# agwi-lab/renderformer

Hardware: AMD Instinct MI355X
Metric: rendered frames/sec at 512×512, renderformer-v1.1-swin-large, 1/2/4/8 MI355X (higher is better)
Workload: dtype fp16+bf16

## Files before the change

### renderformer_amd/csrc/gemm.hip

```cpp
#include <algorithm>
#include <type_traits>
#include <cmath>
#include <math.h>
#include <stdio.h>
#include <stdlib.h>
#include <string.h>

#include "common.h"
#include "env.h"

namespace {

constexpr int BK = 32;
constexpr int P_F16 = 2;

enum Epi { E_BF16 = RF_EPI_BF16, E_F32 = RF_EPI_F32, E_ADD = RF_EPI_ADD_F32, E_SWIGLU = RF_EPI_SWIGLU, E_CONV = 16,
           E_ROPE = 17 };

template <int BM_, int BN_, int WGM_, int WGN_, int STAGES_, int KH_ = 1>
struct Tile {
    static constexpr int BM = BM_, BN = BN_, WGM = WGM_, WGN = WGN_, STAGES = STAGES_, KH = KH_;
    static constexpr int NWAVE = WGM * WGN, THREADS = NWAVE * 64;
    static constexpr int MW = BM / WGM, NWD = BN / WGN, TI = MW / 16, TJ = NWD / 16;
    static constexpr int APIECES = BM / 16;
// ... 1790 lines not shown
            wait_vm<0>();
            __syncthreads();
            if (kf == 0) pn_issue<C, EPI>(p, area, m0, n0);
            engine_mainloop<C, NTERM, GATHER, EPI == E_ADD>(p, smem, m0, n0, kf, kl, acc);
            if (kf != 0) {
                const __amdgpu_buffer_rsrc_t rs = __builtin_amdgcn_make_buffer_rsrc(
                    p.sk_part + (int64_t)L * (BM * BN), 0, BM * BN * 4, 0x00020000);
#pragma unroll
                for (int i = 0; i < TI; ++i)
#pragma unroll
                    for (int j = 0; j < TJ; ++j) {
                        const int off = (((wave * TI + i) * TJ + j) * 64 + lane) * 16;
                        __builtin_amdgcn_raw_buffer_store_b128(__builtin_bit_cast(u32x4, acc[i][j]), rs, off, 0, 16);
                    }
                asm volatile("s_waitcnt vmcnt(0)" ::: "memory");
                __syncthreads();
                if (threadIdx.x == 0) __hip_atomic_store(p.sk_flag + L, p.sk_epoch, __ATOMIC_RELAXED, __HIP_MEMORY_SCOPE_AGENT);
            } else {
                if (kl < iters) {
                    const int64_t tile_end = (int64_t)(tile + 1) * iters;
                    for (int c = L + 1; c < gend; ++c) {
                        int64_t cb, ce;
                        lay.equal_range(c, grp, ntiles64, iters, cb, ce);
                        if (cb >= tile_end) break;
                        if (ce == cb) continue;
                        if (threadIdx.x == 0) {
                            int spins = 0;
                            while (__hip_atomic_load(p.sk_flag + c, __ATOMIC_RELAXED, __HIP_MEMORY_SCOPE_AGENT) != p.sk_epoch &&
                                   ++spins < p.spin)
                                __builtin_amdgcn_s_sleep(1);
                            if (spins >= p.spin) report_device_error(p.err, RF_DEVERR_SK_GEMM);
                            __builtin_amdgcn_fence(__ATOMIC_ACQUIRE, "agent");
                            asm volatile("s_waitcnt vmcnt(0)" ::: "memory");
                        }
                        __syncthreads();
                        const float4* src =
                            reinterpret_cast<const float4*>(p.sk_part + (int64_t)c * (BM * BN)) + wave * TI * TJ * 64 + lane;
#pragma unroll
                        for (int i = 0; i < TI; ++i)
#pragma unroll
                            for (int j = 0; j < TJ; ++j) {
                                const float4 v = src[(i * TJ + j) * 64];
                                acc[i][j][0] += v.x;
                                acc[i][j][1] += v.y;
                                acc[i][j][2] += v.z;
                                acc[i][j][3] += v.w;
                            }
                    }
                }
                engine_epilogue<C, EPI>(p, m0, n0, acc, area);
            }
            it += kl - kf;
        }
    }
}

constexpr int GROUP_MAX = 4;
struct GroupArgs {
    EngineArgs p[GROUP_MAX];
    int first[GROUP_MAX + 1];
    int n;
};

template <class C, int EPI, int NTERM, bool GATHER>
__global__ __launch_bounds__(C::THREADS, 2) void engine_group_kernel(GroupArgs g) {
    constexpr int BM = C::BM, BN = C::BN, TI = C::TI, TJ = C::TJ;
    __shared__ __attribute__((aligned(16))) char smem[C::STAGES * stage_bytes<C, NTERM>()];
    const int nwg = gridDim.x, hw = blockIdx.x;
    const int xcd = hw & 7, qd = nwg >> 3, rd = nwg & 7;
    const int wg = (xcd < rd ? xcd * (qd + 1) : rd * (qd + 1) + (xcd - rd) * qd) + (hw >> 3);
    int q = 0;
#pragma unroll
    for (int i = 1; i < GROUP_MAX; ++i) q += (i < g.n && wg >= g.first[i]) ? 1 : 0;
    const EngineArgs& p = g.p[q];
    const int local = wg - g.first[q];
    const int tiles_m = (p.m + BM - 1) / BM;
    int tm, tn;
    tile_coords(local, tiles_m, p.n / BN, p.group_m, tm, tn);
    f32x4 acc[TI][TJ];
    engine_mainloop<C, NTERM, GATHER, EPI == E_ADD>(p, smem, tm * BM, tn * BN, 0, p.k / (BK * C::KH), acc);
    engine_epilogue<C, EPI>(p, tm * BM, tn * BN, acc);
}

template <class C>
struct Halo {
    static constexpr int ROWS = (3 * (C::BM + 2) + 15) / 16 * 16;
    static constexpr int BYTES = ROWS * 64;
    static constexpr int PIECES = ROWS / 16;
    static constexpr int PPW = (PIECES + C::NWAVE - 1) / C::NWAVE;
    static constexpr int BST = 3;
    static constexpr int LDS = 2 * BYTES + BST * C::B_BYTES;
};

template <class C>
RF_DEV void halo_mainloop(const EngineArgs& p, char* smem, int m0, int n0, f32x4 (&acc)[C::TI][C::TJ]) {
    using H = Halo<C>;
    constexpr int TI = C::TI, TJ = C::TJ, PB = C::PB, S = H::BST;
    const int lane = threadIdx.x & 63;
    const int wave = threadIdx.x >> 6;
    const int wm = wave / C::WGN, wn = wave % C::WGN;
    const int lg = p.halo_lg, tw = 1 << lg, hw2 = tw + 2;
    const int hr_n = ((C::BM >> lg) + 2) * hw2;
    const int per_img = p.ho * p.wo;
    const int img = m0 / per_img, rem = m0 - img * per_img;
    const int y0 = rem / p.wo, x0 = rem - y0 * p.wo;

    int hpix[H::PPW];
#pragma unroll
    for (int t = 0; t < H::PPW; ++t) {
        const int hr = (wave + C::NWAVE * t) * 16 + (lane >> 2);
        int pix = -1;
        if (hr < hr_n) {
            const int hy = hr / hw2, hx = hr - hy * hw2;
            const int iy = y0 + hy - 1, ix = x0 + hx - 1;
            if (iy >= 0 && iy < p.hi && ix >= 0 && ix < p.wi) pix = (img * p.hi + iy) * p.wi + ix;
        }
        hpix[t] = pix;
    }
    int brow[PB], blc[PB];
#pragma unroll
    for (int pc = 0; pc < PB; ++pc) {
        brow[pc] = (wave * PB + pc) * 16 + (lane >> 2);
        blc[pc] = (lane & 3) ^ ((brow[pc] >> 1) & 3);
    }
    auto issue_halo = [&](int chunk, int buf) {
#pragma unroll
        for (int t = 0; t < H::PPW; ++t) {
            const int piece = wave + C::NWAVE * t;
            if (piece < H::PIECES) {
                const int hch = (lane & 3) ^ (((piece * 16 + (lane >> 2)) >> 1) & 3);
                const bf16_t* src = hpix[t] >= 0 ? p.a + (int64_t)hpix[t] * p.cin_pad + chunk * BK + hch * 8 : p.zero;
                __builtin_amdgcn_global_load_lds(GLB_PTR(void, src), LDS_PTR(void, smem + buf * H::BYTES + piece * 1024),
                                                 16, 0, 0);
            }
        }
    };
    auto issue_w = [&](int kt, int stage) {
        const int chunk = kt / 9, tap = kt - 9 * chunk;
        const int k0 = tap * p.cin_pad + chunk * BK;
        char* st = smem + 2 * H::BYTES + stage * C::B_BYTES;
#pragma unroll
        for (int pc = 0; pc < PB; ++pc) {
            const int piece = wave * PB + pc;
            const int64_t woff = (int64_t)(n0 + brow[pc]) * p.ldw + k0 + blc[pc] * 8;
            __builtin_amdgcn_global_load_lds(GLB_PTR(void, p.w + woff), LDS_PTR(void, st + piece * 1024), 16, 0, 0);
        }
    };

#pragma unroll
    for (int i = 0; i < TI; ++i)
#pragma unroll
        for (int j = 0; j < TJ; ++j) acc[i][j] = f32x4{0.f, 0.f, 0.f, 0.f};

    const int nch = p.cin_pad / BK, nk = 9 * nch;
    const int frag_row = lane & 15, frag_ch = lane >> 4;
    auto base_hr = [&](int i) {
        const int r = wm * C::MW + i * 16 + frag_row;
        return r + ((r >> lg) << 1);
    };
    struct Frags {
        bf16x8 a[TI], w[TJ];
    };
    auto load_frags = [&](int kt, Frags& f) {
        const int chunk = kt / 9, tap = kt - 9 * chunk;
        const int ky = tap / 3, kx = tap - 3 * ky;
        const char* hb = smem + (chunk & 1) * H::BYTES;
// ... 762 lines not shown
    RF_LAUNCH((engine_kernel<C, EPI, NTERM, GATHER, true>), dim3(grid), dim3(C::THREADS), 0,
                       (hipStream_t)stream, a);
    return rf::check_launch(what);
}

int sk_setup(EngineArgs& p, void* workspace, void* stream) {
    p.sk_part = (float*)workspace;
    p.sk_flag = (int*)(p.sk_part + SK_PART_FLOATS);
    p.sk_epoch = rf::next_epoch(p.sk_flag, SK_MAX_GRID * sizeof(int), (hipStream_t)stream);
    if (p.sk_epoch == 0) return RF_ERR_LAUNCH;
    p.err = rf::device_error_word();
    p.spin = rf::spin_limit();
    p.stamps = RF_ENV_ONCE("RF_GEMM_STAMPS", 0) != 0 ? (uint64_t*)(p.sk_part + SK_PART_FLOATS - 65536) : nullptr;
    return RF_OK;
}

template <class F>
int with_epi(int epilogue, F&& f) {
    switch (epilogue) {
        case RF_EPI_BF16: return f(std::integral_constant<int, E_BF16>{});
        case RF_EPI_F32: return f(std::integral_constant<int, E_F32>{});
        case RF_EPI_ADD_F32: return f(std::integral_constant<int, E_ADD>{});
        default: return f(std::integral_constant<int, E_SWIGLU>{});
    }
}

inline void dense_args(EngineArgs& p, const void* a, int64_t lda, const void* w, int64_t ldw, int m, int n, int k,
                       void* c, int64_t ldc) {
    p.a = (const bf16_t*)a;
    p.lda = lda;
    p.w = (const bf16_t*)w;
    p.ldw = ldw;
    p.m = m;
    p.n = n;
    p.k = k;
    p.c = c;
    p.ldc = ldc;
}


int sk_grid(int m, int n, int k) {
    const bool env = rf::env_set("RF_GEMM_SK");
    int grid = 2 * 256;
    if (!env) return 0;
    if (env) {
        grid = rf::env_int("RF_GEMM_SK", 0);
        if (grid <= 0) return 0;
        grid = grid > SK_MAX_GRID ? SK_MAX_GRID : grid;
    }
    const int64_t tiles = (int64_t)((m + 127) / 128) * (n / 128);
    const int64_t rounds = (tiles + 511) / 512;
    const double eff = (double)tiles / (rounds * 512);
    if (!env && (eff >= 0.9 || tiles * (k / BK) < 8LL * grid)) return 0;
    return grid;
}

enum TileCode : int {
    TC_R128 = 128,
    TC_P256 = 256,
    TC_P288 = 288,
    TC_R64 = 642,
    TC_P64 = 643,
    TC_R64w4 = 644,
    TC_P3_64 = 645,
    TC_R64s6 = 646,
    TC_R96 = 962,
    TC_P96 = 963,
    TC_P3_96 = 964,
    TC_R96s5 = 965,
    TC_R96s6 = 966,
    TC_P128 = 1282,
    TC_P3_128 = 1283,
    TC_R128s4 = 1284,
    TC_R128s5 = 1285,
    TC_R128s6 = 1286,
    TC_R128w8s6 = 1288,
    TC_R256x128 = 2561,
    TC_R64k2 = 6423,
    TC_R64w4k2 = 6443,
    TC_R96k2 = 9623,
    TC_R128k2s3 = 12823,
    TC_R128k2s4 = 12824,
    TC_R128w8k2 = 12884,
};

int pick_cfg(int m, int n, int k, int epilogue = RF_EPI_BF16) {
    if (rf::env_set("RF_GEMM_TILE")) return rf::env_int("RF_GEMM_TILE", 0);
    const bool phased = n % 256 == 0 && k % 64 == 0 && rf::env_int("RF_GEMM_PHASED", 1) != 0;
    const double kk = k / 1024.0;
    const bool add = epilogue == RF_EPI_ADD_F32;
    auto cost = [&](int bm, int bn, int slots, double fixed, double per_k, double add_cost) {
        const int64_t tiles = (int64_t)((m + bm - 1) / bm) * (n / bn);
        const int64_t rounds = (tiles + 256 * slots - 1) / (256 * slots);
        return rounds * (fixed + per_k * kk + (add ? add_cost : 0.0));
    };
    int best = TC_R128;
    const int64_t t128 = (int64_t)((m + 127) / 128) * (n / 128);
    double best_c = t128 <= 256 ? cost(128, 128, 1, 5.5, 13.1, 5.0) : cost(128, 128, 2, 11.0, 14.0, 5.0);
    auto consider = [&](int cfg, double c) {
        if (c < best_c) {
            best_c = c;
            best = cfg;
        }
    };
    if (k % 64 == 0) consider(TC_R128w8k2, cost(128, 128, 1, 6.8, 10.9, 5.0));
    if (n % 256 == 0) consider(TC_R96, cost(96, 256, 1, 2.2, 16.5, 13.0));
    if (phased) {
        consider(TC_P256, cost(256, 256, 1, 11.0, 20.4, 5.0));
        consider(TC_P288, cost(288, 256, 1, 22.5, 22.1, 5.0));
        consider(TC_P128, cost(128, 256, 1, 2.3, 18.4, 5.0));
        consider(TC_P3_96, cost(96, 256, 1, 6.0, 14.4, 5.0));
        consider(TC_P3_64, cost(64, 256, 1, 6.5, 11.8, 5.0));
    }
    return best;
}

__device__ __attribute__((aligned(16))) bf16_t g_zero_row[64];

namespace mx {
constexpr int BM = 256, BN = 256, KS = 128;
constexpr int A_DATA = BM * KS, B_DATA = BN * KS;
constexpr int STAGE = A_DATA + B_DATA + (BM + BN) * 4;
constexpr int TI = 8, TJ = 4;
typedef __attribute__((ext_vector_type(8))) int i32x8;
RF_DEV int off(int row, int ch) { return row * KS + ((ch ^ (row & 7)) << 4); }
}

template <bool INITC>
RF_DEV void mx8_mainloop(const EngineArgs& p, char* smem, int m0, int n0, int kbeg, int kend,
                         f32x4 (&acc)[mx::TI][mx::TJ]) {
    using namespace mx;
    const int lane = threadIdx.x & 63;
    const int wave = threadIdx.x >> 6;
    const int wm = wave >> 2, wn = wave & 3;
    const int nk = kend - kbeg;
    const uint8_t* A = reinterpret_cast<const uint8_t*>(p.a);
    const uint8_t* W = reinterpret_cast<const uint8_t*>(p.w);
    auto issue = [&](int kt, int buf) {
        char* st = smem + buf * STAGE;
        const int64_t k0 = (int64_t)(kbeg + kt) * KS;
#pragma unroll
        for (int i = 0; i < 8; ++i) {
            const int piece = wave * 8 + i;
            const bool is_a = piece < BM / 8;
            const int row = (is_a ? piece : piece - BM / 8) * 8 + (lane >> 3);
            const int ch = (lane & 7) ^ (row & 7);
            const uint8_t* src;
            if (is_a) {
                const int m = m0 + row;
                src = A + (int64_t)(m < p.m ? m : p.m - 1) * p.lda + k0 + ch * 16;
            } else {
                src = W + (int64_t)(n0 + row) * p.ldw + k0 + ch * 16;
            }
            __builtin_amdgcn_global_load_lds(GLB_PTR(void, src), LDS_PTR(void, st + (is_a ? 0 : A_DATA) + piece % (BM / 8) * 1024),
                                             16, 0, 0);
        }
        {
            const bool is_a = wave < BM / 64;
            const int row = (is_a ? wave : wave - BM / 64) * 64 + lane;
            const uint8_t* src;
            if (is_a) {
                const int m = m0 + row;
                src = p.sa + (int64_t)(m < p.m ? m : p.m - 1) * p.ld_sa + (kbeg + kt) * 4;
            } else {
                src = p.sw + (int64_t)(n0 + row) * p.ld_sw + (kbeg + kt) * 4;
            }
            __builtin_amdgcn_global_load_lds(GLB_PTR(void, src),
                                             LDS_PTR(void, st + A_DATA + B_DATA + (is_a ? 0 : BM * 4) + (row & ~63) * 4),
                                             4, 0, 0);
        }
    };
    if (INITC && kbeg == 0) {
        load_c_acc<TI, TJ>(p, m0 + wm * 128, n0 + wn * 64, acc);
    } else {
#pragma unroll
        for (int i = 0; i < TI; ++i)
#pragma unroll
            for (int j = 0; j < TJ; ++j) acc[i][j] = f32x4{0.f, 0.f, 0.f, 0.f};
    }
    const int frow = lane & 15, g = lane >> 4;
    issue(0, 0);
    if (nk > 1) {
        issue(1, 1);
        wait_vm<9>();
    } else {
        wait_vm<0>();
    }
    __builtin_amdgcn_s_barrier();
// ... 217 lines not shown
    int e = -127;
    if (amax > 0.f) {
        int ex;
        const float f = frexpf(amax, &ex);
        e = ex - 9 + (f > 0.875f ? 1 : 0);
        e = e < -127 ? -127 : (e > 127 ? 127 : e);
    }
    const float inv = ldexpf(1.0f, -e);
    uint32_t out[8];
#pragma unroll
    for (int i = 0; i < 8; ++i) {
        int pk = __builtin_amdgcn_cvt_pk_fp8_f32(v[4 * i] * inv, v[4 * i + 1] * inv, 0, false);
        pk = __builtin_amdgcn_cvt_pk_fp8_f32(v[4 * i + 2] * inv, v[4 * i + 3] * inv, pk, true);
        out[i] = (uint32_t)pk;
    }
    uint4* dst = reinterpret_cast<uint4*>(q + (int64_t)row * ldq + b * 32);
    dst[0] = make_uint4(out[0], out[1], out[2], out[3]);
    dst[1] = make_uint4(out[4], out[5], out[6], out[7]);
    sc[(int64_t)row * lds + b] = (uint8_t)(e + 127);
}

}

bool persist_on() {
    return RF_ENV_ONCE("RF_GEMM_PERSIST", 1) != 0;
}

bool persist_ragged() {
    return RF_ENV_ONCE("RF_GEMM_PERSIST_RAGGED", 0) != 0;
}

template <int EPI, int NTERM, bool GATHER, int BM = 256>
int launch_phased(EngineArgs a, void* stream, const char* what) {
    const int tiles_m = (a.m + BM - 1) / BM, tiles_n = a.n / 256;
    const int nwg = tiles_n * tiles_m;
    a.group_m = pick_group_m(tiles_m, tiles_n, BM, 256, (nwg + 7) / 8, GATHER ? 0 : (int64_t)a.m * a.k * 2);
    if constexpr (BM == 256 && (NTERM == 1 || NTERM == P_F16) && !GATHER) {
        if (nwg > 256 && persist_on() && (nwg % 256 == 0 || persist_ragged())) {
            a.persist = 1;
            RF_LAUNCH((phased_sk_kernel<EPI, NTERM>), dim3(256), dim3(512), 0, (hipStream_t)stream, a);
            return rf::check_launch(what);
        }
    }
    RF_LAUNCH((phased_kernel<BM, EPI, NTERM, GATHER>), dim3(nwg), dim3(512), 0, (hipStream_t)stream, a);
    return rf::check_launch(what);
}

#ifdef RF_STUDY
int l2pf_dist() {
    return std::max(0, std::min(8, rf::env_int("RF_GEMM_L2PF", 0)));
}
#endif

template <int EPI, int BM, int NT = 1>
int launch_phased3(EngineArgs a, void* stream, const char* what) {
#ifdef RF_STUDY
    a.l2pf = l2pf_dist();
#endif
    const int tiles_m = (a.m + BM - 1) / BM, tiles_n = a.n / 256;
    const int nwg = tiles_n * tiles_m;
    a.group_m = pick_group_m(tiles_m, tiles_n, BM, 256, (nwg + 7) / 8, (int64_t)a.m * a.k * 2);
    RF_LAUNCH((phased3_kernel<BM, EPI, NT>), dim3(nwg), dim3(512), 0, (hipStream_t)stream, a);
    return rf::check_launch(what);
}

template <int EPI, int NT = 1>
int launch_phased_sk(EngineArgs a, int grid, void* stream, const char* what) {
    const int tiles_m = (a.m + 255) / 256, tiles_n = a.n / 256;
    a.group_m = pick_group_m(tiles_m, tiles_n, 256, 256, ((int64_t)tiles_m * tiles_n + 7) / 8);
    RF_LAUNCH((phased_sk_kernel<EPI, NT>), dim3(grid), dim3(512), 0, (hipStream_t)stream, a);
    return rf::check_launch(what);
}

bool use_phased(int n, int k) {
    return rf::env_int("RF_GEMM_PHASED", 1) != 0 && n % 256 == 0 && k % 64 == 0;
}

template <class C>
struct Ring {};
template <int BM>
struct Phased {};
template <int BM>
struct Phased3 {};

enum Pre { PRE_NONE = 0, PRE_N256 = 1, PRE_K64 = 2, PRE_PHASED = 4 };

bool pre_ok(int pre, const EngineArgs& p) {
    return (!(pre & PRE_N256) || p.n % 256 == 0) && (!(pre & PRE_K64) || p.k % 64 == 0) &&
           (!(pre & PRE_PHASED) || use_phased(p.n, p.k));
}

template <int CODE, class LOOP, int PRE, bool F16>
struct Row {};
template <class... R>
struct Rows {};

using TileTable = Rows<
    Row<TC_P256,        Phased<256>,                      PRE_PHASED,          true>,
    Row<TC_P128,        Phased<128>,                      PRE_PHASED,          true>,
    Row<TC_P288,        Phased<288>,                      PRE_PHASED,          true>,
    Row<TC_P256,        Ring<T256>,                       PRE_N256,            false>,
    Row<TC_R128s4,      Ring<Tile<128, 128, 2, 2, 4>>,    PRE_NONE,            false>,
    Row<TC_R128s5,      Ring<Tile<128, 128, 2, 2, 5>>,    PRE_NONE,            false>,
    Row<TC_R256x128,    Ring<T256x128>,                   PRE_NONE,            false>,
    Row<TC_R96,         Ring<T96x256>,                    PRE_N256,            true>,
    Row<TC_R64,         Ring<T64x256>,                    PRE_N256,            false>,
    Row<TC_P3_128,      Phased3<128>,                     PRE_PHASED,          true>,
    Row<TC_P3_96,       Phased3<96>,                      PRE_PHASED,          true>,
    Row<TC_P3_64,       Phased3<64>,                      PRE_PHASED,          true>,
    Row<TC_P96,         Phased<96>,                       PRE_PHASED,          false>,
    Row<TC_P64,         Phased<64>,                       PRE_PHASED,          false>,
    Row<TC_R64w4,       Ring<T64x256w4>,                  PRE_N256,            false>,
    Row<TC_R96s5,       Ring<T96x256s5>,                  PRE_N256,            false>,
    Row<TC_R96s6,       Ring<T96x256s6>,                  PRE_N256,            false>,
    Row<TC_R64s6,       Ring<T64x256s6>,                  PRE_N256,            false>,
    Row<TC_R128s6,      Ring<T128s6>,                     PRE_NONE,            false>,
    Row<TC_R128w8s6,    Ring<T128w8s6>,                   PRE_NONE,            false>,
    Row<TC_R128k2s3,    Ring<T128k2s3>,                   PRE_K64,             false>,
    Row<TC_R128k2s4,    Ring<T128k2s4>,                   PRE_K64,             false>,
    Row<TC_R128w8k2,    Ring<T128w8k2s4>,                 PRE_K64,             true>,
    Row<TC_R96k2,       Ring<T96x256k2>,                  PRE_K64 | PRE_N256,  false>,
    Row<TC_R64k2,       Ring<T64x256k2>,                  PRE_K64 | PRE_N256,  false>,
    Row<TC_R64w4k2,     Ring<T64x256w4k2>,                PRE_K64 | PRE_N256,  false>,
    Row<TC_R128,        Ring<T128>,                       PRE_NONE,            true>>;

template <int NT, class C>
int run_loop(Ring<C>, const EngineArgs& p, int epilogue, void* stream) {
    return with_epi(epilogue, [&](auto e) { return launch<C, decltype(e)::value, NT>(p, stream, "rf_gemm"); });
}
template <int NT, int BM>
int run_loop(Phased<BM>, const EngineArgs& p, int epilogue, void* stream) {
    return with_epi(epilogue, [&](auto e) {
        return launch_phased<decltype(e)::value, NT, false, BM>(p, stream, NT == P_F16 ? "rf_gemm_f16" : "rf_gemm_bf16");
    });
}
template <int NT, int BM>
int run_loop(Phased3<BM>, const EngineArgs& p, int epilogue, void* stream) {
    return with_epi(epilogue, [&](auto e) { return launch_phased3<decltype(e)::value, BM, NT>(p, stream, "rf_gemm"); });
}

template <int NT, int CODE, class LOOP, int PRE, bool F16>
bool try_row(Row<CODE, LOOP, PRE, F16>, int cfg, const EngineArgs& p, int epilogue, void* stream, int& rc) {
    if constexpr (NT == P_F16 && !F16) {
        return false;
    } else {
        if (cfg != CODE || !pre_ok(PRE, p)) return false;
        rc = run_loop<NT>(LOOP{}, p, epilogue, stream);
        return true;
    }
}

template <int NT, class... R>
int run_dp(Rows<R...>, int cfg, const EngineArgs& p, int epilogue, void* stream) {
    int rc = RF_OK;
    if ((try_row<NT>(R{}, cfg, p, epilogue, stream, rc) || ...)) return rc;
    return run_loop<NT>(Ring<T128>{}, p, epilogue, stream);
}

bool sk256(int m, int n, int k) { return rf::env_int("RF_GEMM_SK256", 0) != 0; }

bool skph(int m, int n, int k) {
    if (!use_phased(n, k)) return false;
    if (rf::env_set("RF_GEMM_SKPH")) return rf::env_int("RF_GEMM_SKPH", 0) != 0;
    const int64_t tiles = (int64_t)((m + 255) / 256) * (n / 256);
    return n % 256 == 0 && tiles >= 512 && tiles % 256 == 0;
}

extern "C" int64_t rf_gemm_workspace_bytes(void) { return SK_WS_BYTES; }

#ifdef RF_STUDY
static int quad_tile() {
    const char* env = rf::env_str("RF_GEMM_QUAD_TILE");
    if (!env) return 256256;
    int bm = 0, bn = 0;
    if (sscanf(env, "%dx%d", &bm, &bn) != 2) return 256256;
    return bm * 1000 + bn;
}

static int quad_mode(int m, int n, int k, int64_t lda, int64_t ldw, int epilogue) {
    const int mode = rf::env_int("RF_GEMM_QUAD", 0);
    if (mode <= 0 || k % 128 || m <= 0) return 0;
    const int t = quad_tile(), bn = t % 1000;
    if (bn != 256 && bn != 192 && bn != 128) return 0;
    if (epilogue == RF_EPI_SWIGLU && n % bn) return 0;
    if ((int64_t)m * lda * 2 >= 0x7fffffff || (int64_t)n * ldw * 2 >= 0x7fffffff) return 0;
    return mode;
}

template <int WM, int WN, int EPI, int NT, int STG>
static int launch_quad_s(EngineArgs a, int mode, void* workspace, int64_t ws_bytes, void* stream, const char* what);

template <int WM, int WN, int EPI, int NT>
static int launch_quad(EngineArgs a, int mode, void* workspace, int64_t ws_bytes, void* stream, const char* what) {
    if (rf::env_int("RF_GEMM_QUAD_STG", 0) == 1) return launch_quad_s<WM, WN, EPI, NT, 1>(a, mode, workspace, ws_bytes, stream, what);
    return launch_quad_s<WM, WN, EPI, NT, 0>(a, mode, workspace, ws_bytes, stream, what);
}

template <int WM, int WN, int EPI, int NT, int STG>
static int launch_quad_s(EngineArgs a, int mode, void* workspace, int64_t ws_bytes, void* stream, const char* what) {
    using G = qd::Cfg<WM, WN>;
    const int tiles_m = (a.m + G::BM - 1) / G::BM, tiles_n = (a.n + G::BN - 1) / G::BN;
    const int64_t tiles = (int64_t)tiles_m * tiles_n;
    const int grid = (int)std::min<int64_t>(tiles, 256);
    a.group_m = pick_group_m(tiles_m, tiles_n, G::BM, G::BN, (grid + 7) / 8);
    if (mode == 2 && workspace && ws_bytes >= SK_WS_BYTES) {
        if (const int rc = sk_setup(a, workspace, stream)) return rc;
        RF_LAUNCH((quad_kernel<WM, WN, EPI, NT, STG>), dim3(256), dim3(256), 0, (hipStream_t)stream, a);
    } else {
        a.sk_flag = nullptr;
        RF_LAUNCH((quad_kernel<WM, WN, EPI, NT, STG>), dim3(grid), dim3(256), 0, (hipStream_t)stream, a);
    }
    return rf::check_launch(what);
}

template <int WM, int WN, int NT>
static int run_quad_t(const EngineArgs& p, int epilogue, int mode, void* workspace, int64_t ws_bytes, void* stream,
                      const char* what) {
    return with_epi(epilogue, [&](auto e) {
        return launch_quad<WM, WN, decltype(e)::value, NT>(p, mode, workspace, ws_bytes, stream, what);
    });
}
// ... 98 lines not shown
    nio.xg = (bf16_t*)xg;
    nio.ldxg = ldxg;
    nio.norm_g = norm_w;
    nio.ss_out = ss;
    nio.xg_f16 = f16;
    return gemm_bf16(a, lda, w, ldw, x, ldx, nullptr, m, n, k, RF_EPI_ADD_F32, workspace, ws_bytes, stream, nullptr,
                     f16, &nio);
}

extern "C" int rf_gemm_rownorm(const void* a, int64_t lda, const void* w, int64_t ldw, void* c, int64_t ldc, int m,
                               int n, int k, int epilogue, const float* ss, int norm_dim, float eps, float* seg_ss,
                               int seg_w, int n_seg, int operand_dtype, void* workspace, int64_t ws_bytes,
                               void* stream) {
    RF_REQUIRE(ss && ((uintptr_t)ss & 15) == 0, "rf_gemm_rownorm: ss must be 16-B aligned");
    RF_REQUIRE(norm_dim > 0, "rf_gemm_rownorm: norm_dim must be positive");
    RF_REQUIRE(epilogue == RF_EPI_BF16 || epilogue == RF_EPI_F16 || epilogue == RF_EPI_SWIGLU ||
                   epilogue == RF_EPI_SWIGLU_F16,
               "rf_gemm_rownorm: epilogue must be RF_EPI_BF16 / F16 / SWIGLU / SWIGLU_F16 (got %d)", epilogue);
    RF_REQUIRE(operand_dtype == RF_DT_F16 || operand_dtype == RF_DT_BF16, "rf_gemm_rownorm: operand_dtype");
    RF_REQUIRE(!seg_ss || ((epilogue == RF_EPI_BF16 || epilogue == RF_EPI_F16) && ((uintptr_t)seg_ss & 15) == 0 &&
                           seg_w > 0 && seg_w % 256 == 0 && seg_w <= PN_SLOTS * 128 && n_seg >= 1 &&
                           (int64_t)seg_w * n_seg <= n),
               "rf_gemm_rownorm: seg_ss needs a 16-bit (non-SwiGLU) epilogue, 16-B alignment, seg_w %% 256 == 0 and "
               "<= %d, n_seg >= 1 segments inside N", PN_SLOTS * 128);
    EngineArgs nio{};
    nio.rs_part = ss;
    nio.rs_n = (float)norm_dim;
    nio.rs_eps = eps;
    nio.seg_ss = seg_ss;
    nio.seg_w = seg_w;
    nio.seg_n = seg_ss ? n_seg : 0;
    return gemm_bf16(a, lda, w, ldw, c, ldc, nullptr, m, n, k, epilogue, workspace, ws_bytes, stream, nullptr,
                     operand_dtype == RF_DT_F16, &nio);
}

template <class C, int NT>
static int launch_rope(EngineArgs p, void* stream) {
    return launch<C, E_ROPE, NT>(p, stream, "rf_gemm_qk_rope");
}

extern "C" int rf_gemm_qk_rope(const void* a, int64_t lda, const void* w, int64_t ldw, void* c, int64_t ldc, int m,
                               int n, int k, const float* ss, int norm_dim, float eps, float* seg_ss, int seg_w,
                               int n_seg, const float* norm_w, const float* pos, int64_t ld_pos, int pos_div,
                               const float* freqs, int n_freqs, float q_scale, int operand_dtype, void* workspace,
                               int64_t ws_bytes, void* stream) {
    (void)workspace;
    (void)ws_bytes;
    RF_REQUIRE(a && w && c, "rf_gemm_qk_rope: null pointer");
    RF_REQUIRE(m > 0 && n > 0 && k > 0, "rf_gemm_qk_rope: empty problem m=%d n=%d k=%d", m, n, k);
    RF_REQUIRE(operand_dtype == RF_DT_F16 || operand_dtype == RF_DT_BF16, "rf_gemm_qk_rope: operand_dtype");
    RF_REQUIRE(k % 64 == 0 && n % 128 == 0, "rf_gemm_qk_rope: needs K %% 64 == 0 and N %% 128 == 0");
    RF_REQUIRE(lda % 8 == 0 && ldw % 8 == 0 && lda >= k && ldw >= k && ((uintptr_t)a & 15) == 0 &&
                   ((uintptr_t)w & 15) == 0, "rf_gemm_qk_rope: operands must be 16-B aligned with lda/ldw >= K");
    RF_REQUIRE(ldc >= n && ldc % 4 == 0 && ((uintptr_t)c & 7) == 0, "rf_gemm_qk_rope: ldc too small/unaligned");
    RF_REQUIRE(seg_w > 0 && seg_w % 256 == 0 && seg_w % 128 == 0 && n_seg >= 1 && (int64_t)seg_w * n_seg <= n,
               "rf_gemm_qk_rope: the q/k segments must be whole 256-column tiles inside N");
    RF_REQUIRE(!seg_ss || (((uintptr_t)seg_ss & 15) == 0 && seg_w <= PN_SLOTS * 128),
               "rf_gemm_qk_rope: seg_ss must be 16-B aligned and seg_w <= %d", PN_SLOTS * 128);
    RF_REQUIRE(!ss || (((uintptr_t)ss & 15) == 0 && norm_dim > 0), "rf_gemm_qk_rope: ss must be 16-B aligned");
    RF_REQUIRE(!norm_w || ((uintptr_t)norm_w & 15) == 0, "rf_gemm_qk_rope: norm_w must be 16-B aligned");
    RF_REQUIRE(!pos || (freqs && n_freqs > 0 && 9 * n_freqs <= 64 && ld_pos >= 9 && pos_div >= 1),
               "rf_gemm_qk_rope: pos needs freqs with 9 * n_freqs <= 64, ld_pos >= 9 and pos_div >= 1");
    EngineArgs p{};
    dense_args(p, a, lda, w, ldw, m, n, k, c, ldc);
    p.rs_part = ss;
    p.rs_n = (float)norm_dim;
    p.rs_eps = eps;
    p.seg_ss = norm_w ? seg_ss : nullptr;
    p.seg_w = seg_w;
    p.seg_n = n_seg;
    p.rope_pos = pos;
    p.rope_ld = ld_pos;
    p.rope_div = pos ? pos_div : 1;
    p.rope_freqs = freqs;
    p.rope_nf = pos ? n_freqs : 1;
    p.rope_g = norm_w;
    p.rope_qscale = q_scale;
    const bool f16 = operand_dtype == RF_DT_F16;
    const int cfg = pick_cfg(m, n, k, RF_EPI_BF16);
    if (cfg == TC_P288 && use_phased(n, k)) {
        return f16 ? launch_phased<E_ROPE, P_F16, false, 288>(p, stream, "rf_gemm_qk_rope")
                   : launch_phased<E_ROPE, 1, false, 288>(p, stream, "rf_gemm_qk_rope");
    }
    const bool t96 = n % 256 == 0 && cfg != TC_R128w8k2;
    if (t96) return f16 ? launch_rope<T96x256, P_F16>(p, stream) : launch_rope<T96x256, 1>(p, stream);
    return f16 ? launch_rope<T128w8k2s4, P_F16>(p, stream) : launch_rope<T128w8k2s4, 1>(p, stream);
}

extern "C" int rf_gemm_bf16_if(const int* flag, const void* a, int64_t lda, const void* w, int64_t ldw, void* c,
                               int64_t ldc, const float* bias, int m, int n, int k, int epilogue, void* workspace,
                               int64_t ws_bytes, void* stream) {
    RF_REQUIRE(flag, "rf_gemm_bf16_if: null flag");
    return gemm_bf16(a, lda, w, ldw, c, ldc, bias, m, n, k, epilogue, workspace, ws_bytes, stream, flag);
}

extern "C" int rf_gemm_mx8(const void* a, int64_t lda, const void* sa, int64_t ld_sa, const void* w, int64_t ldw,
                           const void* sw, int64_t ld_sw, void* c, int64_t ldc, const float* bias, int m, int n, int k,
                           int epilogue, void* stream) {
    RF_REQUIRE(a && w && sa && sw && c, "rf_gemm_mx8: null pointer");
    RF_REQUIRE(m > 0 && n > 0 && k > 0, "rf_gemm_mx8: empty problem");
    RF_REQUIRE(k % 128 == 0 && n % 256 == 0, "rf_gemm_mx8: K=%d must be a multiple of 128 and N=%d of 256", k, n);
    RF_REQUIRE(lda % 16 == 0 && ldw % 16 == 0 && lda >= k && ldw >= k, "rf_gemm_mx8: lda/ldw (bytes) >= K, 16-B aligned");
    RF_REQUIRE(ld_sa % 4 == 0 && ld_sw % 4 == 0 && ld_sa >= k / 32 && ld_sw >= k / 32,
               "rf_gemm_mx8: scale rows must hold K/32 bytes, 4-B aligned");
    RF_REQUIRE(((uintptr_t)a & 15) == 0 && ((uintptr_t)w & 15) == 0 && ((uintptr_t)sa & 3) == 0 && ((uintptr_t)sw & 3) == 0,
               "rf_gemm_mx8: operands 16-B / scales 4-B aligned");
    RF_REQUIRE(epilogue >= RF_EPI_BF16 && epilogue <= RF_EPI_SWIGLU, "rf_gemm_mx8: bad epilogue %d", epilogue);
    RF_REQUIRE(ldc >= (epilogue == RF_EPI_SWIGLU ? n / 2 : n) && ldc % 4 == 0, "rf_gemm_mx8: ldc too small/unaligned");
    EngineArgs p{};
    dense_args(p, a, lda, w, ldw, m, n, k, c, ldc);
    p.sa = (const uint8_t*)sa;
    p.sw = (const uint8_t*)sw;
    p.ld_sa = (int)ld_sa;
    p.ld_sw = (int)ld_sw;
    p.bias = bias;
    hipStream_t st = (hipStream_t)stream;
    if (RF_ENV_ONCE("RF_MX8_PLAIN", 0) == 0) {
        const int tiles_m = (m + 127) / 128, tiles_n = n / 256;
        const int nwg = tiles_m * tiles_n;
        p.group_m = pick_group_m(tiles_m, tiles_n, 128, 256, (nwg + 7) / 8, (int64_t)m * k);
        const dim3 g(nwg), b(512);
        return with_epi(epilogue, [&](auto e) {
            RF_LAUNCH((mx8_p3_kernel<decltype(e)::value>), g, b, 0, st, p);
            return rf::check_launch("rf_gemm_mx8");
        });
    }
    const int tiles_m = (m + 255) / 256, tiles_n = n / 256;
    const int nwg = tiles_m * tiles_n;
    p.group_m = pick_group_m(tiles_m, tiles_n, 256, 256, (nwg + 7) / 8, (int64_t)m * k);
    const dim3 g(nwg), b(512);
    return with_epi(epilogue, [&](auto e) {
        RF_LAUNCH((mx8_kernel<decltype(e)::value>), g, b, 0, st, p);
        return rf::check_launch("rf_gemm_mx8");
    });
}

extern "C" int rf_quant_mx8(const void* x, int64_t ldx, int rows, int cols, void* q, int64_t ldq, void* scales,
                            int64_t ld_s, void* stream) {
    RF_REQUIRE(x && q && scales, "rf_quant_mx8: null pointer");
    RF_REQUIRE(cols % 32 == 0 && ldx % 8 == 0 && ldq % 16 == 0 && ldq >= cols && ld_s >= cols / 32,
               "rf_quant_mx8: cols %% 32, 16-B rows");
    if (rows <= 0) return RF_OK;
    const int64_t n = (int64_t)rows * (cols / 32);
    RF_LAUNCH(quant_mx8_kernel, dim3((unsigned)((n + 255) / 256)), dim3(256), 0, (hipStream_t)stream,
                       (const bf16_t*)x, ldx, rows, cols, (uint8_t*)q, ldq, (uint8_t*)scales, ld_s);
    return rf::check_launch("rf_quant_mx8");
}

static bool halo2_ok(const EngineArgs& a) {
    const int env = rf::env_int("RF_CONV_HALO2", -1);
    if (env == 0) return false;
    if (!rf::env_set("RF_CONV_HALO2") && rf::env_set("RF_CONV_TILE")) return false;
    if (a.kw != 3 || a.k != 9 * a.cin_pad || a.stride != 1 || a.pad != 1 || a.ho != a.hi || a.wo != a.wi) return false;
    if (a.cin_pad % 32 || (a.n % 128 && a.n != 64) || a.ho % h2::TH || a.wo % h2::TW || a.m % 512) return false;
    const int64_t blocks = (int64_t)(a.m / 512) * (a.n == 64 ? 1 : a.n / 128);
    return env == 1 || blocks >= 256;
}

static int launch_halo2(EngineArgs a, void* stream, const char* what) {
    const bool n64 = a.n == 64;
    const int nwg = (a.m / 512) * (n64 ? 1 : a.n / 128);
    const int ring = rf::env_int("RF_CONV_H2S", 4);
    const hipStream_t st = (hipStream_t)stream;
    const int dbg = rf::env_int("RF_H2_DBG", 0);
#ifndef RF_STUDY
    if (dbg) return rf::study_only("rf_conv: RF_H2_DBG (halo2 ablation builds)");
#else
// ... 423 lines not shown
```

Measured before the change: 95.63.

## Add hand-scheduled inline-asm 128x128 GEMM mainloop with interleaved loads and MFMA

Adds a new 128x128 GEMM kernel whose mainloop is written in inline assembly. It interleaves global loads, LDS writes, LDS reads and MFMA instructions, using s_setprio and explicit waitcnts with double-buffered LDS. The cost model selects this tile when K is a multiple of 128 and it scores cheaper than the existing 128-tile options, and the QK-RoPE path can also use it. The goal is to hide memory latency behind matrix math better than the compiler-scheduled ring loop. The price is hard-coded register allocation (v176-v255 clobbered), fragility, and the chance that the cost model picks this tile for shapes where it is slower.

```diff
diff --git a/renderformer_amd/csrc/gemm.hip b/renderformer_amd/csrc/gemm.hip
--- a/renderformer_amd/csrc/gemm.hip
+++ b/renderformer_amd/csrc/gemm.hip
@@ -1896,6 +1896,151 @@
     engine_epilogue<C, EPI>(p, tm * BM, tn * BN, acc);
 }
 
+#define HS_S(i) "v[176+4*(" #i "):179+4*(" #i ")]"
+#define HS_FA(b, i) "v[208+24*" #b "+4*" #i ":211+24*" #b "+4*" #i "]"
+#define HS_FW(b, j) "v[224+24*" #b "+4*" #j ":227+24*" #b "+4*" #j "]"
+#define HS_WAITVM(n) "s_waitcnt vmcnt(" #n ")\n\t"
+#define HS_WAITLGKM(n) "s_waitcnt lgkmcnt(" #n ")\n\t"
+#define HS_GLD_A(h) "global_load_dwordx4 " HS_S(h) ", %[voffA], %[sA] offset:64*" #h "\n\t"
+#define HS_GLD_W(h) "global_load_dwordx4 " HS_S(4+h) ", %[voffW], %[sW] offset:64*" #h "\n\t"
+#define HS_DSW_A(h) "ds_write_b128 %[wr], " HS_S(h) " offset:8192*" #h "\n\t"
+#define HS_DSW_W(h) "ds_write_b128 %[wr], " HS_S(4+h) " offset:32768+8192*" #h "\n\t"
+#define HS_ADV_A "v_add_u32 %[voffA], 0x100, %[voffA]\n\t"
+#define HS_ADV_W "v_add_u32 %[voffW], 0x100, %[voffW]\n\t"
+#define HS_LOAD_STEP HS_GLD_A(0) HS_GLD_A(1) HS_GLD_A(2) HS_GLD_A(3) HS_ADV_A HS_GLD_W(0) HS_GLD_W(1) HS_GLD_W(2) HS_GLD_W(3) HS_ADV_W
+#define HS_PA_FULL(h, n) HS_WAITVM(7) HS_DSW_A(h) HS_GLD_A(h)
+#define HS_PW_FULL(h, n) HS_WAITVM(7) HS_DSW_W(h) HS_GLD_W(h)
+#define HS_PA_WR(h, n) HS_WAITVM(n) HS_DSW_A(h)
+#define HS_PW_WR(h, n) HS_WAITVM(n) HS_DSW_W(h)
+#define HS_PA_NONE(h, n)
+#define HS_PW_NONE(h, n)
+#define HS_ADV_FULL(x) x
+#define HS_ADV_WR(x)
+#define HS_ADV_NONE(x)
+#define HS_RD_A(b, i, h) "ds_read_b128 " HS_FA(b, i) ", %[rdA] offset:8192*" #h "+1024*" #i "\n\t"
+#define HS_RD_W(b, j, h) "ds_read_b128 " HS_FW(b, j) ", %[rdW] offset:8192*" #h "+1024*" #j "\n\t"
+#define HS_RD_ALL(b, h) HS_RD_A(b, 0, h) HS_RD_A(b, 1, h) HS_RD_A(b, 2, h) HS_RD_A(b, 3, h) HS_RD_W(b, 0, h) HS_RD_W(b, 1, h)
+#define HS_MFMA(MF, b, i, j) MF " %[a" #i #j "], " HS_FW(b, j) ", " HS_FA(b, i) ", %[a" #i #j "]\n\t"
+#define HS_MM(MF, b, i) HS_MFMA(MF, b, i, 0) HS_MFMA(MF, b, i, 1)
+#define HS_SLICE_RD(MF, b, h2, P0, P1, P2, P3)                                                                     \
+    "s_setprio 1\n\t" HS_MM(MF, b, 0) HS_RD_A(b, 0, h2) P0 HS_MM(MF, b, 1) HS_RD_A(b, 1, h2) P1 HS_MM(MF, b, 2)    \
+    HS_RD_A(b, 2, h2) P2 HS_MM(MF, b, 3) "s_setprio 0\n\t" HS_RD_A(b, 3, h2) HS_RD_W(b, 0, h2) HS_RD_W(b, 1, h2) P3
+#define HS_SLICE(MF, b) "s_setprio 1\n\t" HS_MM(MF, b, 0) HS_MM(MF, b, 1) HS_MM(MF, b, 2) HS_MM(MF, b, 3) "s_setprio 0\n\t"
+#define HS_STEP(MF, V, L01, MID)                                                                                   \
+    HS_RD_ALL(1, 1) HS_WAITLGKM(6)                                                                                 \
+    HS_SLICE_RD(MF, 0, 2, HS_PA_##V(0, 7), HS_PA_##V(1, 6), HS_PA_##V(2, 5), HS_PA_##V(3, 4) HS_ADV_##V(HS_ADV_A)) \
+    HS_WAITLGKM(L01)                                                                                               \
+    HS_SLICE_RD(MF, 1, 3, HS_PW_##V(0, 3), HS_PW_##V(1, 2), HS_PW_##V(2, 1), HS_PW_##V(3, 0) HS_ADV_##V(HS_ADV_W)) \
+    HS_WAITLGKM(L01) HS_SLICE(MF, 0) MID HS_SLICE(MF, 1)
+#define HS_TOGGLE "v_xor_b32 %[rdA], %[tA], %[rdA]\n\tv_xor_b32 %[rdW], %[tW], %[rdW]\n\tv_xor_b32 %[wr], %[tw], %[wr]\n\t"
+#define HS_PUBLISH "s_waitcnt lgkmcnt(0)\n\ts_barrier\n\t"
+#define HS_NEXT HS_PUBLISH HS_TOGGLE HS_RD_ALL(0, 0)
+#define HS_LOAD_C(i) "global_load_dwordx4 %[a" #i "0], %[c" #i "], off\n\tglobal_load_dwordx4 %[a" #i "1], %[c" #i "], off offset:64\n\t"
+#define HS_LOOP(MF)                                                                                                 \
+    HS_LOAD_STEP                                                                           \
+    "s_cmp_lt_u32 %[cnt], 2\n\ts_cbranch_scc1 1f\n\t"                                                               \
+    HS_PA_FULL(0, 7) HS_PA_FULL(1, 7) HS_PA_FULL(2, 7) HS_PA_FULL(3, 7) HS_ADV_A  \
+    HS_PW_FULL(0, 7) HS_PW_FULL(1, 7) HS_PW_FULL(2, 7) HS_PW_FULL(3, 7) HS_ADV_W "s_branch 2f\n"                    \
+    "1:\n\t" HS_PA_WR(0, 7) HS_PA_WR(1, 6) HS_PA_WR(2, 5) HS_PA_WR(3, 4) HS_PW_WR(0, 3) HS_PW_WR(1, 2) HS_PW_WR(2, 1) \
+    HS_PW_WR(3, 0) "\n2:\n\t" HS_PUBLISH "v_xor_b32 %[wr], %[tw], %[wr]\n\t" HS_RD_ALL(0, 0)                        \
+    "s_cmp_lt_u32 %[cnt], 3\n\ts_cbranch_scc1 4f\n"                                                                 \
+    "3:\n\t" HS_STEP(MF, FULL, 10, HS_NEXT)                                                                         \
+    "s_sub_u32 %[cnt], %[cnt], 1\n\ts_cmp_ge_u32 %[cnt], 3\n\ts_cbranch_scc1 3b\n"                                  \
+    "4:\n\ts_cmp_lt_u32 %[cnt], 2\n\ts_cbranch_scc1 5f\n\t" HS_STEP(MF, WR, 10, HS_NEXT)                            \
+    "\n5:\n\t" HS_STEP(MF, NONE, 6, HS_WAITLGKM(0))  \
+    "s_nop 15\n\ts_nop 3"
+#define HS_CLOB10(a) "v" #a "0", "v" #a "1", "v" #a "2", "v" #a "3", "v" #a "4", "v" #a "5", "v" #a "6", "v" #a "7", "v" #a "8", "v" #a "9"
+
+constexpr int HS_STAGE = 2 * 4 * 128 * 64;
+using THs = Tile<128, 128, 2, 4, 4, 2>;
+
+template <int NTERM, bool INITC>
+RF_DEV void engine_mainloop_hs(const EngineArgs& p, char* smem, int m0, int n0, f32x4 (&acc)[4][2]) {
+    static_assert(NTERM == 1 || NTERM == P_F16, "hs: bf16 or fp16 operands");
+    const int lane = threadIdx.x & 63;
+    const int wave = threadIdx.x >> 6;
+    const int wm = wave >> 2, wn = wave & 3;
+    const int srow = wave * 16 + (lane >> 2);
+    const int sch = (lane & 3) ^ ((srow >> 1) & 3);
+    const int arow = min(m0 + srow, p.m - 1) - m0;
+    uint32_t voffA = (uint32_t)arow * (uint32_t)p.lda * 2u + sch * 16;
+    uint32_t voffW = (uint32_t)srow * (uint32_t)p.ldw * 2u + sch * 16;
+    const bf16_t* sA = p.a + (int64_t)m0 * p.lda;
+    const bf16_t* sW = p.w + (int64_t)n0 * p.ldw;
+    const uint32_t lds0 = lds_addr(smem);
+    uint32_t wr = lds0 + wave * 1024 + lane * 16;
+    uint32_t rdA = lds0 + lds_off(wm * 64 + (lane & 15), lane >> 4);
+    uint32_t rdW = lds0 + 4 * 8192 + lds_off(wn * 32 + (lane & 15), lane >> 4);
+    const uint32_t tw = wr ^ (wr + HS_STAGE), tA = rdA ^ (rdA + HS_STAGE), tW = rdW ^ (rdW + HS_STAGE);
+    int cnt = p.k / 128;
+#pragma unroll
+    for (int i = 0; i < 4; ++i)
+#pragma unroll
+        for (int j = 0; j < 2; ++j) acc[i][j] = f32x4{0.f, 0.f, 0.f, 0.f};
+#define HS_OPERANDS                                                                                                 \
+    [a00] "+v"(acc[0][0]), [a01] "+v"(acc[0][1]), [a10] "+v"(acc[1][0]), [a11] "+v"(acc[1][1]),                     \
+    [a20] "+v"(acc[2][0]), [a21] "+v"(acc[2][1]), [a30] "+v"(acc[3][0]), [a31] "+v"(acc[3][1]),                     \
+    [voffA] "+v"(voffA), [voffW] "+v"(voffW), [wr] "+v"(wr), [rdA] "+v"(rdA), [rdW] "+v"(rdW), [cnt] "+s"(cnt)
+#define HS_CLOBBERS                                                                                                 \
+    "memory", "scc", "v176", "v177", "v178", "v179", HS_CLOB10(18), HS_CLOB10(19), HS_CLOB10(20), HS_CLOB10(21),        \
+    HS_CLOB10(22), HS_CLOB10(23), HS_CLOB10(24), "v250", "v251", "v252", "v253", "v254", "v255"
+    if constexpr (INITC) {
+        const float* crow[4];
+#pragma unroll
+        for (int i = 0; i < 4; ++i) {
+            const int row = min(m0 + wm * 64 + i * 16 + (lane & 15), p.m - 1);
+            crow[i] = reinterpret_cast<const float*>(p.c) + (int64_t)row * p.ldc + n0 + wn * 32 + 4 * (lane >> 4);
+        }
+        if constexpr (NTERM == P_F16)
+            asm volatile("s_nop 4\n\t" HS_LOAD_C(0) HS_LOAD_C(1) HS_LOAD_C(2) HS_LOAD_C(3) HS_LOOP("v_mfma_f32_16x16x32_f16")
+                         : HS_OPERANDS
+                         : [sA] "s"(sA), [sW] "s"(sW), [tw] "v"(tw), [tA] "v"(tA), [tW] "v"(tW), [c0] "v"(crow[0]),
+                           [c1] "v"(crow[1]), [c2] "v"(crow[2]), [c3] "v"(crow[3])
+                         : HS_CLOBBERS);
+        else
+            asm volatile("s_nop 4\n\t" HS_LOAD_C(0) HS_LOAD_C(1) HS_LOAD_C(2) HS_LOAD_C(3) HS_LOOP("v_mfma_f32_16x16x32_bf16")
+                         : HS_OPERANDS
+                         : [sA] "s"(sA), [sW] "s"(sW), [tw] "v"(tw), [tA] "v"(tA), [tW] "v"(tW), [c0] "v"(crow[0]),
+                           [c1] "v"(crow[1]), [c2] "v"(crow[2]), [c3] "v"(crow[3])
+                         : HS_CLOBBERS);
+    } else {
+        if constexpr (NTERM == P_F16)
+            asm volatile("s_nop 4\n\t" HS_LOOP("v_mfma_f32_16x16x32_f16")
+                         : HS_OPERANDS
+                         : [sA] "s"(sA), [sW] "s"(sW), [tw] "v"(tw), [tA] "v"(tA), [tW] "v"(tW)
+                         : HS_CLOBBERS);
+        else
+            asm volatile("s_nop 4\n\t" HS_LOOP("v_mfma_f32_16x16x32_bf16")
+                         : HS_OPERANDS
+                         : [sA] "s"(sA), [sW] "s"(sW), [tw] "v"(tw), [tA] "v"(tA), [tW] "v"(tW)
+                         : HS_CLOBBERS);
+    }
+#undef HS_OPERANDS
+#undef HS_CLOBBERS
+}
+
+template <int EPI, int NTERM>
+__global__ __launch_bounds__(512, 1) void hs128_kernel(EngineArgs p) {
+    using C = THs;
+    constexpr int MAIN = 2 * HS_STAGE;
+    static_assert(MAIN + PN_AREA<C, EPI> <= 160 * 1024, "hs: LDS budget");
+    __shared__ __attribute__((aligned(16))) char smem[MAIN + PN_AREA<C, EPI>];
+    char* const area = smem + MAIN;
+    if (gated_off(p)) return;
+    const int tiles_m = (p.m + 127) / 128;
+    const int nwg = gridDim.x;
+    const int hw = blockIdx.x;
+    const int xcd = hw & 7, q = nwg >> 3, r = nwg & 7;
+    const int wg = (xcd < r ? xcd * (q + 1) : r * (q + 1) + (xcd - r) * q) + (hw >> 3);
+    int tm, tn;
+    tile_coords(wg, tiles_m, p.n / 128, p.group_m, tm, tn);
+    const int m0 = tm * 128, n0 = tn * 128;
+    f32x4 acc[4][2];
+    pn_issue<C, EPI>(p, area, m0, n0);
+    engine_mainloop_hs<NTERM, EPI == E_ADD>(p, smem, m0, n0, acc);
+    engine_epilogue<C, EPI>(p, m0, n0, acc, area);
+}
+
 template <class C>
 struct Halo {
     static constexpr int ROWS = (3 * (C::BM + 2) + 15) / 16 * 16;
@@ -2824,6 +2969,7 @@
     TC_R128k2s3 = 12823,
     TC_R128k2s4 = 12824,
     TC_R128w8k2 = 12884,
+    TC_H128 = 12885,
 };
 
 int pick_cfg(int m, int n, int k, int epilogue = RF_EPI_BF16) {
@@ -2846,6 +2992,7 @@
         }
     };
     if (k % 64 == 0) consider(TC_R128w8k2, cost(128, 128, 1, 6.8, 10.9, 5.0));
+    if (k % 128 == 0) consider(TC_H128, cost(128, 128, 1, 6.5, 9.9, 5.0));
     if (n % 256 == 0) consider(TC_R96, cost(96, 256, 1, 2.2, 16.5, 13.0));
     if (phased) {
         consider(TC_P256, cost(256, 256, 1, 11.0, 20.4, 5.0));
@@ -3229,12 +3376,17 @@
 struct Phased {};
 template <int BM>
 struct Phased3 {};
-
-enum Pre { PRE_NONE = 0, PRE_N256 = 1, PRE_K64 = 2, PRE_PHASED = 4 };
+struct Hs128 {};
+
+enum Pre { PRE_NONE = 0, PRE_N256 = 1, PRE_K64 = 2, PRE_PHASED = 4, PRE_HS = 8 };
+
+bool hs_ok(const EngineArgs& p) {
+    return p.k % 128 == 0 && p.n % 128 == 0 && p.lda < (1 << 23) && p.ldw < (1 << 23);
+}
 
 bool pre_ok(int pre, const EngineArgs& p) {
     return (!(pre & PRE_N256) || p.n % 256 == 0) && (!(pre & PRE_K64) || p.k % 64 == 0) &&
-           (!(pre & PRE_PHASED) || use_phased(p.n, p.k));
+           (!(pre & PRE_PHASED) || use_phased(p.n, p.k)) && (!(pre & PRE_HS) || hs_ok(p));
 }
 
 template <int CODE, class LOOP, int PRE, bool F16>
@@ -3266,6 +3418,7 @@
     Row<TC_R128k2s3,    Ring<T128k2s3>,                   PRE_K64,             false>,
     Row<TC_R128k2s4,    Ring<T128k2s4>,                   PRE_K64,             false>,
     Row<TC_R128w8k2,    Ring<T128w8k2s4>,                 PRE_K64,             true>,
+    Row<TC_H128,        Hs128,                            PRE_HS,              true>,
     Row<TC_R96k2,       Ring<T96x256k2>,                  PRE_K64 | PRE_N256,  false>,
     Row<TC_R64k2,       Ring<T64x256k2>,                  PRE_K64 | PRE_N256,  false>,
     Row<TC_R64w4k2,     Ring<T64x256w4k2>,                PRE_K64 | PRE_N256,  false>,
@@ -3284,6 +3437,19 @@
 template <int NT, int BM>
 int run_loop(Phased3<BM>, const EngineArgs& p, int epilogue, void* stream) {
     return with_epi(epilogue, [&](auto e) { return launch_phased3<decltype(e)::value, BM, NT>(p, stream, "rf_gemm"); });
+}
+
+template <int EPI, int NT>
+int launch_hs(EngineArgs a, void* stream, const char* what) {
+    const int tiles_m = (a.m + 127) / 128, tiles_n = a.n / 128;
+    const int nwg = tiles_n * tiles_m;
+    a.group_m = pick_group_m(tiles_m, tiles_n, 128, 128, (nwg + 7) / 8, (int64_t)a.m * a.k * 2);
+    RF_LAUNCH((hs128_kernel<EPI, NT>), dim3(nwg), dim3(512), 0, (hipStream_t)stream, a);
+    return rf::check_launch(what);
+}
+template <int NT>
+int run_loop(Hs128, const EngineArgs& p, int epilogue, void* stream) {
+    return with_epi(epilogue, [&](auto e) { return launch_hs<decltype(e)::value, NT>(p, stream, "rf_gemm"); });
 }
 
 template <int NT, int CODE, class LOOP, int PRE, bool F16>
@@ -3548,7 +3714,10 @@
         return f16 ? launch_phased<E_ROPE, P_F16, false, 288>(p, stream, "rf_gemm_qk_rope")
                    : launch_phased<E_ROPE, 1, false, 288>(p, stream, "rf_gemm_qk_rope");
     }
-    const bool t96 = n % 256 == 0 && cfg != TC_R128w8k2;
+    if (cfg == TC_H128 && hs_ok(p)) {
+        return f16 ? launch_hs<E_ROPE, P_F16>(p, stream, "rf_gemm_qk_rope") : launch_hs<E_ROPE, 1>(p, stream, "rf_gemm_qk_rope");
+    }
+    const bool t96 = n % 256 == 0 && cfg != TC_R128w8k2 && cfg != TC_H128;
     if (t96) return f16 ? launch_rope<T96x256, P_F16>(p, stream) : launch_rope<T96x256, 1>(p, stream);
     return f16 ? launch_rope<T128w8k2s4, P_F16>(p, stream) : launch_rope<T128w8k2s4, 1>(p, stream);
 }
```

Result: no change. 96.34 (median of 6 runs) (+0.7%).
